# HKUST-Aerial-Robotics/VINS-Mobile

Hardware: AMD Instinct MI355X
Metric: VIO frames/sec (KLT+window solve), 640x480/150 feats/W=10 (higher is better)
Workload: dtype f64 (solve) / u8+i32+f32 (KLT)

## Files before the change

### vins-mobile_amd/csrc/vio_frontend.hip

```cpp
#include <hip/hip_runtime.h>

#include <type_traits>

#include "vio_exact_math.h"

#include <math.h>
#include <stdint.h>
#include <stdio.h>
#include <string.h>

#include <algorithm>
#include <condition_variable>
#include <memory>
#include <mutex>
#include <thread>
#include <vector>

#include "vio_amd.h"
#include "vio_device.h"
#include "vio_pool.h"

namespace {

constexpr int kMaxLevels = 4;
constexpr int kMaxCap = 512;
constexpr int kWin = 21;
constexpr int kWBits = 14;
constexpr int kMaxRadius = 128;

struct LevelDims {
  int rows[kMaxLevels], cols[kMaxLevels];
  size_t off[kMaxLevels];
  size_t pyr_bytes;
  int levels;
};

__device__ __forceinline__ int reflect101(int p, int len) {
  p = p < 0 ? -p : p;
  p = p >= len ? 2 * len - 2 - p : p;
  return p;
}
__device__ __forceinline__ int descale(int x, int n) { return (x + (1 << (n - 1))) >> n; }

constexpr int kPdW = 64, kPdH = 8;
__global__ __launch_bounds__(256) void pyr_down_kernel(const uint8_t *src_base, uint8_t *dst_base, size_t seq_stride,
                                                       int srows, int scols, int drows, int dcols) {
  constexpr int SW = 2 * kPdW + 4, SH = 2 * kPdH + 4;
  __shared__ int patch[SH][SW + 1];
  __shared__ int hsum[SH][kPdW + 1];
  const uint8_t *src = src_base + (size_t)blockIdx.z * seq_stride;
  uint8_t *dst = dst_base + (size_t)blockIdx.z * seq_stride;
  const int ox = blockIdx.x * kPdW, oy = blockIdx.y * kPdH;
  const int tid = threadIdx.x;
  for (int e = tid; e < SH * SW; e += 256) {
    int ly = e / SW, lx = e - ly * SW;
    int y = reflect101(min(2 * oy + ly - 2, 2 * srows - 2), srows), x = reflect101(min(2 * ox + lx - 2, 2 * scols - 2), scols);
    patch[ly][lx] = src[(size_t)y * scols + x];
  }
  __syncthreads();
  for (int e = tid; e < SH * kPdW; e += 256) {
    int ly = e / kPdW, lx = e - ly * kPdW;
    const int *r = &patch[ly][2 * lx];
    hsum[ly][lx] = r[0] + 4 * r[1] + 6 * r[2] + 4 * r[3] + r[4];
  }
  __syncthreads();
  for (int e = tid; e < kPdH * kPdW; e += 256) {
    int ly = e / kPdW, lx = e - ly * kPdW;
    int x = ox + lx, y = oy + ly;
    if (x < dcols && y < drows) {
      int v = hsum[2 * ly][lx] + 4 * hsum[2 * ly + 1][lx] + 6 * hsum[2 * ly + 2][lx] + 4 * hsum[2 * ly + 3][lx] + hsum[2 * ly + 4][lx];
      dst[(size_t)y * dcols + x] = (uint8_t)((v + 128) >> 8);
    }
  }
}

inline float lk_eps_screen(double eps_sq) { return nextafterf((float)(eps_sq * (1.0 + 1e-5)), INFINITY); }
struct LkParams {
  LevelDims ld;
  int cap;
  int max_count;
  float epsilon_sq_f;
  double epsilon_sq;
  float min_eig;
  const uint8_t *prev0, *next0;
  size_t stride0;
};

__device__ __forceinline__ int wave_sum_i32(int v) {
  v += __builtin_amdgcn_update_dpp(0, v, 0x111, 0xf, 0xf, false);
  v += __builtin_amdgcn_update_dpp(0, v, 0x112, 0xf, 0xf, false);
  v += __builtin_amdgcn_update_dpp(0, v, 0x114, 0xf, 0xf, false);
  v += __builtin_amdgcn_update_dpp(0, v, 0x118, 0xf, 0xf, false);
  v += __builtin_amdgcn_update_dpp(0, v, 0x142, 0xa, 0xf, false);
  v += __builtin_amdgcn_update_dpp(0, v, 0x143, 0xc, 0xf, false);
  return __builtin_amdgcn_readlane(v, 63);
}
__device__ __forceinline__ double wave_sum_exact(int p) {
  int lo = p & 0xffff, hi = p >> 16;
  int slo = wave_sum_i32(lo), shi = wave_sum_i32(hi);
  return (double)shi * 65536.0 + (double)slo;
}

__device__ __forceinline__ void lk_weights(float a, float b, int &iw00, int &iw01, int &iw10, int &iw11) {
  iw00 = __float2int_rn((1.f - a) * (1.f - b) * (1 << kWBits));
  iw01 = __float2int_rn(a * (1.f - b) * (1 << kWBits));
  iw10 = __float2int_rn((1.f - a) * b * (1 << kWBits));
  iw11 = (1 << kWBits) - iw00 - iw01 - iw10;
}

constexpr int kIP = kWin + 3;
constexpr int kDP = kWin + 1;
constexpr int kJMargin = 3;
constexpr int kJP = kWin + 1 + 2 * kJMargin;
constexpr int kJS = 43;
constexpr int kIS = kIP + 1;
struct LkWaveLds {
  union {
    struct {
      uint32_t I[kIP][kIS];
      short2 dI[kDP][kDP];
    };
    uint32_t J[kJP][kJS];
  };
};
typedef short lk_s2 __attribute__((ext_vector_type(2)));
typedef unsigned short lk_us2 __attribute__((ext_vector_type(2)));

struct __attribute__((packed)) LkU32 {
  uint32_t v;
};
__device__ __forceinline__ uint32_t lk_load4(const uint8_t *p) { return reinterpret_cast<const LkU32 *>(p)->v; }
__device__ __forceinline__ void lk_pairs(uint32_t cur, uint32_t next, uint32_t w[4]) {
  w[0] = __builtin_amdgcn_perm(0u, cur, 0x0c010c00u);
  w[1] = __builtin_amdgcn_perm(0u, cur, 0x0c020c01u);
  w[2] = __builtin_amdgcn_perm(0u, cur, 0x0c030c02u);
  w[3] = __builtin_amdgcn_perm(next, cur, 0x0c040c03u);
}

__device__ __forceinline__ void wave_lds_fence() {
  __builtin_amdgcn_fence(__ATOMIC_RELEASE, "wavefront");
  __builtin_amdgcn_wave_barrier();
  __builtin_amdgcn_fence(__ATOMIC_ACQUIRE, "wavefront");
}

__device__ __forceinline__ bool wave_all_small(int p, int q, int r = 0) {
  const bool small = (unsigned)(p + (1 << 24)) < (1u << 25) && (unsigned)(q + (1 << 24)) < (1u << 25) && (unsigned)(r + (1 << 24)) < (1u << 25);
  return __builtin_amdgcn_ballot_w64(!small) == 0ull;
}
__device__ __forceinline__ void wave_sum_exact2(int p, int q, float &sp, float &sq) {
  if (wave_all_small(p, q)) {
    int u[2] = {p, q};
#define VIO_DPPS(ctrl, rmask)                                                  \
  {                                                                            \
    const int t0 = __builtin_amdgcn_update_dpp(0, u[0], ctrl, rmask, 0xf, false); \
    const int t1 = __builtin_amdgcn_update_dpp(0, u[1], ctrl, rmask, 0xf, false); \
    u[0] += t0, u[1] += t1;                                                    \
  }
    VIO_DPPS(0x111, 0xf) VIO_DPPS(0x112, 0xf) VIO_DPPS(0x114, 0xf) VIO_DPPS(0x118, 0xf) VIO_DPPS(0x142, 0xa) VIO_DPPS(0x143, 0xc)
#undef VIO_DPPS
    sp = (float)__builtin_amdgcn_readlane(u[0], 63), sq = (float)__builtin_amdgcn_readlane(u[1], 63);
    return;
  }
  int a = p & 0xffff, b = q & 0xffff, c = p >> 16, d = q >> 16;
#define VIO_DPP4(ctrl, rmask)                                              \
  {                                                                        \
    const int ta = __builtin_amdgcn_update_dpp(0, a, ctrl, rmask, 0xf, false); \
    const int tb = __builtin_amdgcn_update_dpp(0, b, ctrl, rmask, 0xf, false); \
    const int tc = __builtin_amdgcn_update_dpp(0, c, ctrl, rmask, 0xf, false); \
    const int td = __builtin_amdgcn_update_dpp(0, d, ctrl, rmask, 0xf, false); \
    a += ta, b += tb, c += tc, d += td;                                    \
  }
  VIO_DPP4(0x111, 0xf) VIO_DPP4(0x112, 0xf) VIO_DPP4(0x114, 0xf) VIO_DPP4(0x118, 0xf) VIO_DPP4(0x142, 0xa) VIO_DPP4(0x143, 0xc)
#undef VIO_DPP4
  const int sa = __builtin_amdgcn_readlane(a, 63), sb = __builtin_amdgcn_readlane(b, 63), sc = __builtin_amdgcn_readlane(c, 63),
            sd = __builtin_amdgcn_readlane(d, 63);
  sp = (float)sc * 65536.f + (float)sa, sq = (float)sd * 65536.f + (float)sb;
}

__device__ __forceinline__ void wave_sum_exact3(int p, int q, int r, float &sp, float &sq, float &sr) {
  if (wave_all_small(p, q, r)) {
    int w[3] = {p, q, r};
#define VIO_DPPS3(ctrl, rmask)                                                                                       \
  {                                                                                                                   \
    int t[3];                                                                                                         \
    _Pragma("unroll") for (int k = 0; k < 3; k++) t[k] = __builtin_amdgcn_update_dpp(0, w[k], ctrl, rmask, 0xf, false); \
    _Pragma("unroll") for (int k = 0; k < 3; k++) w[k] += t[k];                                                       \
  }
    VIO_DPPS3(0x111, 0xf) VIO_DPPS3(0x112, 0xf) VIO_DPPS3(0x114, 0xf) VIO_DPPS3(0x118, 0xf) VIO_DPPS3(0x142, 0xa) VIO_DPPS3(0x143, 0xc)
#undef VIO_DPPS3
    sp = (float)__builtin_amdgcn_readlane(w[0], 63), sq = (float)__builtin_amdgcn_readlane(w[1], 63), sr = (float)__builtin_amdgcn_readlane(w[2], 63);
    return;
  }
  int u[3] = {p, q, r};
#define VIO_DPPN(N, arr, ctrl, rmask)                                               \
  {                                                                                 \
    int t[N];                                                                       \
    _Pragma("unroll") for (int k = 0; k < N; k++) t[k] = __builtin_amdgcn_update_dpp(0, arr[k], ctrl, rmask, 0xf, false); \
    _Pragma("unroll") for (int k = 0; k < N; k++) arr[k] += t[k];                   \
  }
  VIO_DPPN(3, u, 0x111, 0xf) VIO_DPPN(3, u, 0x112, 0xf) VIO_DPPN(3, u, 0x114, 0xf) VIO_DPPN(3, u, 0x118, 0xf)
  int v[6] = {u[0] & 0xffff, u[1] & 0xffff, u[2] & 0xffff, u[0] >> 16, u[1] >> 16, u[2] >> 16};
  VIO_DPPN(6, v, 0x142, 0xa) VIO_DPPN(6, v, 0x143, 0xc)
#undef VIO_DPPN
  int s[6];
#pragma unroll
  for (int k = 0; k < 6; k++) s[k] = __builtin_amdgcn_readlane(v[k], 63);
  sp = (float)s[3] * 65536.f + (float)s[0], sq = (float)s[4] * 65536.f + (float)s[1], sr = (float)s[5] * 65536.f + (float)s[2];
}

template <bool STATS = false>
__global__ __launch_bounds__(256, 6) void lk_track_kernel(const uint8_t *prev_pyr, const uint8_t *next_pyr, LkParams P,
                                                       const int *n_pts, const float *prev_pts, float *next_pts,
                                                       uint8_t *status, float *err, unsigned long long *stats) {
  __shared__ LkWaveLds lds_all[4];
  const int seq = blockIdx.y;
  const int wave = threadIdx.x >> 6, lane = threadIdx.x & 63;
  const int pt = blockIdx.x * (blockDim.x >> 6) + wave;
  if (pt >= n_pts[seq]) return;
  LkWaveLds &L = lds_all[wave];
  const uint8_t *pp = prev_pyr + (size_t)seq * P.ld.pyr_bytes, *np = next_pyr + (size_t)seq * P.ld.pyr_bytes;
  const size_t pidx = ((size_t)seq * P.cap + pt) * 2;
  const float ptx = prev_pts[pidx], pty = prev_pts[pidx + 1];
  const float half = (kWin - 1) * 0.5f;
  const float FLT_SCALE = 1.f / (1 << 20);
  constexpr int NPX = (kWin * kWin + 63) / 64;
  const int wy0 = min(lane / kWin, 2), wx0 = lane % kWin;
  const int joff = wy0 * kJS + wx0;
  bool st = true;
  float er = 0.f;
  float nxx = 0.f, nxy = 0.f;
  const int max_level = P.ld.levels - 1;
  for (int level = max_level; level >= 0; level--) {
    const int rows = P.ld.rows[level], cols = P.ld.cols[level];
    const uint8_t *I = pp + P.ld.off[level], *J = np + P.ld.off[level];
    if (level == 0) {
      if (P.prev0) I = P.prev0 + (size_t)seq * P.stride0;
      if (P.next0) J = P.next0 + (size_t)seq * P.stride0;
    }
    const float scale = __int_as_float((127 - level) << 23);
    float px = ptx * scale, py = pty * scale;
    float qx, qy;
    if (level == max_level) qx = px, qy = py;
    else qx = nxx * 2.f, qy = nxy * 2.f;
    nxx = qx, nxy = qy;
    px -= half, py -= half;
    int ipx = (int)floorf(px), ipy = (int)floorf(py);
    if (ipx < -kWin || ipx >= cols || ipy < -kWin || ipy >= rows) {
      if (level == 0) st = false, er = 0.f;
      continue;
    }
    float a = px - ipx, b = py - ipy;
    int iw00, iw01, iw10, iw11;
    lk_weights(a, b, iw00, iw01, iw10, iw11);
    wave_lds_fence();
    if (ipx >= 1 && ipx + kIP - 1 <= cols && ipy >= 1 && ipy + kIP - 1 <= rows) {
      const int r = lane / 6, d = lane - 6 * r;
      constexpr int TI = (kIP + 9) / 10;
      uint32_t curs[TI];
#pragma unroll
      for (int t = 0; t < TI; t++) {
        const int ly = r + 10 * t;
        curs[t] = lk_load4(I + (unsigned)(__mul24(ipy - 1 + (ly < kIP ? ly : 0), cols) + ipx - 1 + 4 * d));
      }
#pragma unroll
      for (int t = 0; t < TI; t++) {
        const int ly = r + 10 * t;
        const bool ok = lane < 60 && ly < kIP;
        const uint32_t cur = curs[t];
        uint32_t next = (uint32_t)__builtin_amdgcn_update_dpp(0, (int)cur, 0x130, 0xf, 0xf, false);
        if (d == 5) next = cur >> 24;
        uint32_t w4[4];
        lk_pairs(cur, next, w4);
        if (ok) {
#pragma unroll
          for (int k = 0; k < 4; k++) L.I[ly][4 * d + k] = w4[k];
        }
      }
    } else {
      const int lx = lane & 31;
      const int x = reflect101(ipx - 1 + min(lx, kIP - 1), cols);
      constexpr int RPT = 2, TB = kIP / RPT;
      static_assert(kIP % RPT == 0, "whole trips");
      int vs[TB];
#pragma unroll
      for (int t = 0; t < TB; t++) {
        const int s_y0 = __builtin_amdgcn_readfirstlane(ipy) - 1 + RPT * t;
        const int ro_a = reflect101(s_y0, rows) * cols, ro_b = reflect101(s_y0 + 1, rows) * cols;
        vs[t] = I[(unsigned)(((lane >> 5) ? ro_b : ro_a) + x)];
      }
#pragma unroll
      for (int t = 0; t < TB; t++) {
        const int ly = (lane >> 5) + RPT * t, v = vs[t];
        const int vr = __builtin_amdgcn_update_dpp(0, v, 0x130, 0xf, 0xf, false);
        if (lx < kIP) L.I[ly][lx] = (uint32_t)v | ((uint32_t)vr << 16);
      }
    }
    wave_lds_fence();
    constexpr int SEG = 5, NSEG = 5, NCP = kDP / 2;
    static_assert(kDP % 2 == 0 && NCP * NSEG <= 64 && SEG * NSEG >= kDP && kDP >= SEG, "column pairs x segments");
    const bool inside = ipx >= 0 && ipx + kDP <= cols && ipy >= 0 && ipy + kDP <= rows;
    if (lane < NCP * NSEG) {
      const int seg = lane / NCP, cp = lane - NCP * seg, c = 2 * cp;
      const int r0 = seg * SEG < kDP - SEG ? seg * SEG : kDP - SEG;
      const uint32_t *Ip = &L.I[0][0] + (__mul24(r0, kIS) + c);
      uint32_t *Dp = reinterpret_cast<uint32_t *>(&L.dI[0][0]) + (__mul24(r0, kDP) + c);
      const lk_s2 k3 = {3, 3}, k10 = {10, 10};
      auto walk = [&](auto checked) {
        const unsigned ok0 = (unsigned)(ipx + c) < (unsigned)cols, ok1 = (unsigned)(ipx + c + 1) < (unsigned)cols;
        lk_s2 P0[SEG + 2], P1[SEG + 2], P2[SEG + 2];
#pragma unroll
        for (int r = 0; r < SEG + 2; r++)
          __builtin_memcpy(&P0[r], Ip + r * kIS, 4), __builtin_memcpy(&P1[r], Ip + r * kIS + 1, 4), __builtin_memcpy(&P2[r], Ip + r * kIS + 2, 4);
        lk_s2 h[SEG + 2], v[SEG + 2];
#pragma unroll
        for (int r = 0; r < SEG + 2; r++) h[r] = P2[r] - P0[r], v[r] = (P0[r] + P2[r]) * k3 + P1[r] * k10;
#pragma unroll
        for (int r = 2; r < SEG + 2; r++) {
          const lk_s2 dx = (h[r - 2] + h[r]) * k3 + h[r - 1] * k10, dy = v[r] - v[r - 2];
          uint32_t ux, uy;
          __builtin_memcpy(&ux, &dx, 4), __builtin_memcpy(&uy, &dy, 4);
          uint32_t d0 = __builtin_amdgcn_perm(uy, ux, 0x05040100u), d1 = __builtin_amdgcn_perm(uy, ux, 0x07060302u);
          if (decltype(checked)::value) {
            const unsigned rok = (unsigned)(ipy + r0 + r - 2) < (unsigned)rows;
            d0 &= 0u - (ok0 & rok), d1 &= 0u - (ok1 & rok);
          }
          Dp[(r - 2) * kDP] = d0, Dp[(r - 2) * kDP + 1] = d1;
        }
      };
      if (inside) walk(std::false_type{});
      else walk(std::true_type{});
    }
    wave_lds_fence();
    constexpr int NPP = (NPX + 1) / 2;
    const lk_s2 sw_top = {(short)iw00, (short)iw01}, sw_bot = {(short)iw10, (short)iw11};
    lk_s2 IxP[NPP], IyP[NPP];
    int Ic[NPX];
    int p11 = 0, p12 = 0, p22 = 0;
#pragma unroll
    for (int h = 0; h < NPP; h++) IxP[h] = IyP[h] = lk_s2{0, 0};
#pragma unroll
    for (int q = 0; q < NPX; q++) {
      const int y = wy0 + 3 * q, x = wx0;
      lk_s2 it, ib;
      __builtin_memcpy(&it, &L.I[y + 1][x + 1], 4);
      __builtin_memcpy(&ib, &L.I[y + 2][x + 1], 4);
      const int ival = __builtin_amdgcn_sdot2(it, sw_top, __builtin_amdgcn_sdot2(ib, sw_bot, 1 << (kWBits - 5 - 1), false), false) >> (kWBits - 5);
      uint32_t d00, d01, d10, d11;
      __builtin_memcpy(&d00, &L.dI[y][x], 4), __builtin_memcpy(&d01, &L.dI[y][x + 1], 4);
      __builtin_memcpy(&d10, &L.dI[y + 1][x], 4), __builtin_memcpy(&d11, &L.dI[y + 1][x + 1], 4);
      const uint32_t xt = __builtin_amdgcn_perm(d01, d00, 0x05040100u), yt = __builtin_amdgcn_perm(d01, d00, 0x07060302u);
      const uint32_t xb = __builtin_amdgcn_perm(d11, d10, 0x05040100u), yb = __builtin_amdgcn_perm(d11, d10, 0x07060302u);
      lk_s2 sxt, syt, sxb, syb;
      __builtin_memcpy(&sxt, &xt, 4), __builtin_memcpy(&syt, &yt, 4), __builtin_memcpy(&sxb, &xb, 4), __builtin_memcpy(&syb, &yb, 4);
      int ixval = __builtin_amdgcn_sdot2(sxt, sw_top, __builtin_amdgcn_sdot2(sxb, sw_bot, 1 << (kWBits - 1), false), false) >> kWBits;
      int iyval = __builtin_amdgcn_sdot2(syt, sw_top, __builtin_amdgcn_sdot2(syb, sw_bot, 1 << (kWBits - 1), false), false) >> kWBits;
      if (lane >= 3 * kWin) ixval = iyval = 0;
      Ic[q] = (1 << (kWBits - 5 - 1)) - (int)((unsigned)ival << (kWBits - 5));
      if (q & 1) IxP[q >> 1].y = (short)ixval, IyP[q >> 1].y = (short)iyval;
      else IxP[q >> 1].x = (short)ixval, IyP[q >> 1].x = (short)iyval;
      p11 += ixval * ixval, p12 += ixval * iyval, p22 += iyval * iyval;
    }
    float f11, f12, f22;
    wave_sum_exact3(p11, p12, p22, f11, f12, f22);
    float A11 = f11 * FLT_SCALE, A12 = f12 * FLT_SCALE, A22 = f22 * FLT_SCALE;
    float D = A11 * A22 - A12 * A12;
    float minEig = (A22 + A11 - sqrtf((A11 - A22) * (A11 - A22) + 4.f * A12 * A12)) / (2 * kWin * kWin);
    if (minEig < P.min_eig || D < 1.1920929e-07f) {
      if (level == 0) st = false;
      continue;
    }
    D = 1.f / D;
    qx -= half, qy -= half;
    float pdx = 0.f, pdy = 0.f;
    int jox = 0, joy = 0;
    bool j_staged = false;
    auto stage_j = [&](int iqx, int iqy) {
      jox = iqx - kJMargin, joy = iqy - kJMargin;
      wave_lds_fence();
      if (jox >= 0 && jox + kJP <= cols && joy >= 0 && joy + kJP <= rows) {
        const int r = lane / 7, d = lane - 7 * r;
        constexpr int TJ = (kJP + 8) / 9;
        uint32_t curs[TJ];
#pragma unroll
        for (int t = 0; t < TJ; t++) {
          const int ly = r + 9 * t;
          curs[t] = lk_load4(J + (unsigned)(__mul24(joy + (ly < kJP ? ly : 0), cols) + jox + 4 * d));
        }
#pragma unroll
        for (int t = 0; t < TJ; t++) {
          const int ly = r + 9 * t;
          const bool ok = lane < 63 && ly < kJP;
          const uint32_t cur = curs[t];
          uint32_t next = (uint32_t)__builtin_amdgcn_update_dpp(0, (int)cur, 0x130, 0xf, 0xf, false);
          if (d == 6) next = cur >> 24;
          uint32_t w4[4];
          lk_pairs(cur, next, w4);
          if (ok) {
#pragma unroll
            for (int k = 0; k < 4; k++) L.J[ly][4 * d + k] = w4[k];
          }
        }
      } else {
        const int lx = lane & 31;
        const int x = reflect101(min(max(jox + min(lx, kJP - 1), -cols + 1), 2 * cols - 2), cols);
        constexpr int RPT = 2, TB = kJP / RPT;
        static_assert(kJP % RPT == 0, "whole trips");
        int vs[TB];
#pragma unroll
        for (int t = 0; t < TB; t++) {
          const int s_y0 = __builtin_amdgcn_readfirstlane(joy) + RPT * t;
          const int ro_a = reflect101(min(max(s_y0, -rows + 1), 2 * rows - 2), rows) * cols;
          const int ro_b = reflect101(min(max(s_y0 + 1, -rows + 1), 2 * rows - 2), rows) * cols;
          vs[t] = J[(unsigned)(((lane >> 5) ? ro_b : ro_a) + x)];
        }
#pragma unroll
        for (int t = 0; t < TB; t++) {
          const int ly = (lane >> 5) + RPT * t, v = vs[t];
          const int vr = __builtin_amdgcn_update_dpp(0, v, 0x130, 0xf, 0xf, false);
          if (lx < kJP) L.J[ly][lx] = (uint32_t)v | ((uint32_t)vr << 16);
        }
      }
      wave_lds_fence();
      j_staged = true;
    };
    const uint32_t *Jl = &L.J[0][0];
    auto diff_j = [&](int base, int q, lk_us2 wtop, lk_s2 wbot) {
      lk_us2 top;
      lk_s2 bot;
      const int o = base + (joff + 3 * q * kJS);
      const uint32_t t32 = Jl[o], b32 = Jl[o + kJS];
      __builtin_memcpy(&top, &t32, 4);
      __builtin_memcpy(&bot, &b32, 4);
      return __builtin_amdgcn_sdot2(bot, wbot, (int)__builtin_amdgcn_udot2(top, wtop, (unsigned)Ic[q], false), false) >> (kWBits - 5);
    };
    int nit = 0;
    for (int j = 0; j < P.max_count; j++) {
      int iqx = (int)floorf(qx), iqy = (int)floorf(qy);
      if (iqx < -kWin || iqx >= cols || iqy < -kWin || iqy >= rows) {
        if (level == 0) st = false;
        break;
      }
      if (STATS) nit++;
      if (!j_staged || iqx < jox || iqx > jox + 2 * kJMargin || iqy < joy || iqy > joy + 2 * kJMargin) stage_j(iqx, iqy);
      a = qx - iqx, b = qy - iqy;
      lk_weights(a, b, iw00, iw01, iw10, iw11);
      int pb1 = 0, pb2 = 0;
      const lk_us2 wtop = {(unsigned short)iw00, (unsigned short)iw01};
      const lk_s2 wbot = {(short)iw10, (short)iw11};
      const int jbase = __mul24(iqy - joy, kJS) + (iqx - jox);
#pragma unroll
      for (int h = 0; h < NPP; h++) {
        const int d0 = diff_j(jbase, 2 * h, wtop, wbot), d1 = 2 * h + 1 < NPX ? diff_j(jbase, 2 * h + 1, wtop, wbot) : 0;
        const unsigned pk = __builtin_amdgcn_perm((unsigned)d1, (unsigned)d0, 0x05040100u);
        lk_s2 dp;
        __builtin_memcpy(&dp, &pk, 4);
        pb1 = __builtin_amdgcn_sdot2(dp, IxP[h], pb1, false), pb2 = __builtin_amdgcn_sdot2(dp, IyP[h], pb2, false);
      }
      float fb1, fb2;
      wave_sum_exact2(pb1, pb2, fb1, fb2);
      float b1 = fb1 * FLT_SCALE, b2 = fb2 * FLT_SCALE;
      float ddx = (A12 * b2 - A22 * b1) * D, ddy = (A12 * b1 - A11 * b2) * D;
      qx += ddx, qy += ddy;
      nxx = qx + half, nxy = qy + half;
      if (!(ddx * ddx + ddy * ddy > P.epsilon_sq_f) && (double)ddx * ddx + (double)ddy * ddy <= P.epsilon_sq) break;
      constexpr float kCentiUp = 0.010000000707805157f;
      static_assert((double)kCentiUp > 0.01 && (double)0.01f < 0.01, "float neighbours of 0.01");
      if (j > 0 && fabsf(ddx + pdx) < kCentiUp && fabsf(ddy + pdy) < kCentiUp) {
        nxx -= ddx * 0.5f, nxy -= ddy * 0.5f;
        break;
      }
      pdx = ddx, pdy = ddy;
    }
    if (STATS && lane == 0) {
      unsigned long long *sl = stats + ((blockIdx.x + 7 * blockIdx.y) & 63) * 16;
      atomicAdd(sl + level, (unsigned long long)nit);
      atomicAdd(sl + P.ld.levels + level, 1ull);
    }
    if (st && level == 0) {
      float ex = nxx - half, ey = nxy - half;
      int iex = (int)floorf(ex), iey = (int)floorf(ey);
      if (iex < -kWin || iex >= cols || iey < -kWin || iey >= rows) {
        st = false;
        continue;
      }
      if (!j_staged || iex < jox || iex > jox + 2 * kJMargin || iey < joy || iey > joy + 2 * kJMargin) stage_j(iex, iey);
      float aa = ex - iex, bb = ey - iey;
      lk_weights(aa, bb, iw00, iw01, iw10, iw11);
      int pe = 0;
      const lk_us2 wtop = {(unsigned short)iw00, (unsigned short)iw01};
      const lk_s2 wbot = {(short)iw10, (short)iw11};
      const int jbase = __mul24(iey - joy, kJS) + (iex - jox);
#pragma unroll
      for (int q = 0; q < NPX; q++) {
        const int d = abs(diff_j(jbase, q, wtop, wbot));
        pe += lane < 3 * kWin ? d : 0;
      }
      const int se = wave_sum_i32(pe);
      er = (float)se * 1.f / (32 * kWin * kWin);
    }
  }
  if (lane == 0) {
    next_pts[pidx] = nxx, next_pts[pidx + 1] = nxy;
    status[(size_t)seq * P.cap + pt] = st ? 1 : 0;
    err[(size_t)seq * P.cap + pt] = er;
  }
}

__device__ __attribute__((noinline)) double exact_fn(int which, double x) {
  return which == 0 ? vio_xm::acos_cr(x) : which == 1 ? vio_xm::cos_cr(x) : vio_xm::pow_cr(x, 0.333333333333);
}
__device__ int solve_cubic_dev(const double c[4], double r[3], bool exact) {
  double a0 = c[0], a1 = c[1], a2 = c[2], a3 = c[3];
  double x0 = 0, x1 = 0, x2 = 0;
  int n = 0;
  if (a0 == 0) {
    if (a1 == 0) {
      if (a2 == 0) n = a3 == 0 ? -1 : 0;
      else x0 = -a3 / a2, n = 1;
    } else {
      double d = a2 * a2 - 4 * a1 * a3;
      if (d >= 0) {
        d = sqrt(d);
        double q1 = (-a2 + d) * 0.5, q2 = (a2 + d) * -0.5;
        if (fabs(q1) > fabs(q2)) x0 = q1 / a1, x1 = a3 / q1;
        else x0 = q2 / a1, x1 = a3 / q2;
        n = d > 0 ? 2 : 1;
      }
    }
  } else {
    a0 = 1. / a0, a1 *= a0, a2 *= a0, a3 *= a0;
    double Q = (a1 * a1 - 3 * a2) * (1. / 9), R = (2 * a1 * a1 * a1 - 9 * a1 * a2 + 27 * a3) * (1. / 54);
    double Qcubed = Q * Q * Q, d = Qcubed - R * R;
    const double kPi = 3.14159265358979323846;
    if (d >= 0) {
      const double av = R / sqrt(Qcubed);
      double theta = exact ? exact_fn(0, av) : acos(av), sqrtQ = sqrt(Q);
      double t0 = -2 * sqrtQ, t1 = theta * (1. / 3), t2 = a1 * (1. / 3);
      const double g0 = t1, g1 = t1 + (2. * kPi / 3), g2 = t1 + (4. * kPi / 3);
      if (exact) x0 = t0 * exact_fn(1, g0) - t2, x1 = t0 * exact_fn(1, g1) - t2, x2 = t0 * exact_fn(1, g2) - t2;
      else x0 = t0 * cos(g0) - t2, x1 = t0 * cos(g1) - t2, x2 = t0 * cos(g2) - t2;
      n = 3;
    } else {
      d = sqrt(-d);
      double e = exact ? exact_fn(2, d + fabs(R)) : pow(d + fabs(R), 0.333333333333);
      if (R > 0) e = -e;
      x0 = (e + Q / e) - a1 * (1. / 3);
      n = 1;
    }
  }
  r[0] = x0, r[1] = x1, r[2] = x2;
  return n;
}

struct SevenPointWork {
  double a[63], f1[9], f2[9];
  int colperm[10];
};

__device__ __forceinline__ int run7point_group(const float *ms1, const float *ms2, double *fmatrix, SevenPointWork &wk, int l, bool exact) {
  double *a = wk.a, *f1 = wk.f1, *f2 = wk.f2;
  int *colperm = wk.colperm;
  auto group_sync = [] {
    __builtin_amdgcn_fence(__ATOMIC_RELEASE, "wavefront");
    __builtin_amdgcn_wave_barrier();
    __builtin_amdgcn_fence(__ATOMIC_ACQUIRE, "wavefront");
  };
  if (l < 7) {
    double x0 = ms1[2 * l], y0 = ms1[2 * l + 1], x1 = ms2[2 * l], y1 = ms2[2 * l + 1];
    double *row = a + l * 9;
    row[0] = x1 * x0, row[1] = x1 * y0, row[2] = x1, row[3] = y1 * x0, row[4] = y1 * y0, row[5] = y1, row[6] = x0,
    row[7] = y0, row[8] = 1;
  }
  if (l < 9) colperm[l] = l;
  group_sync();
  for (int k = 0; k < 7; k++) {
    double best = -1;
    int bpos = k * 9 + k;
#pragma unroll
    for (int q = 0; q < 4; q++) {
      const int e = l + 16 * q, i = e / 9, j = e - 9 * i;
      if (e < 63 && i >= k && j >= k) {
        const double v = fabs(a[e]);
        if (v > best) best = v, bpos = e;
      }
    }
#pragma unroll
    for (int m = 1; m < 16; m <<= 1) {
      const double ob = __shfl_xor(best, m, 16);
      const int op = __shfl_xor(bpos, m, 16);
      if (ob > best || (ob == best && op < bpos)) best = ob, bpos = op;
    }
    const int pr = bpos / 9, pc = bpos - 9 * pr;
    if (pr != k && l < 9) {
      const double t = a[k * 9 + l];
      a[k * 9 + l] = a[pr * 9 + l], a[pr * 9 + l] = t;
    }
    group_sync();
    if (pc != k) {
      if (l < 7) {
        const double t = a[l * 9 + k];
        a[l * 9 + k] = a[l * 9 + pc], a[l * 9 + pc] = t;
      }
      if (l == 15) {
        const int t = colperm[k];
        colperm[k] = colperm[pc], colperm[pc] = t;
      }
    }
    group_sync();
    const double d = a[k * 9 + k];
    group_sync();
    if (d == 0.0) continue;
    if (l < 9) a[k * 9 + l] /= d;
    group_sync();
    double fv[4], pv[4], av[4];
    int ev[4];
#pragma unroll
    for (int q = 0; q < 4; q++) {
      const int e = l + 16 * q, ii = e / 9, j = e - 9 * ii, i = ii < k ? ii : ii + 1;
      const bool on = e < 54;
      ev[q] = on ? i * 9 + j : -1;
      fv[q] = on ? a[i * 9 + k] : 0.0, pv[q] = on ? a[k * 9 + j] : 0.0, av[q] = on ? a[i * 9 + j] : 0.0;
    }
    group_sync();
#pragma unroll
    for (int q = 0; q < 4; q++)
      if (ev[q] >= 0 && fv[q] != 0.0) a[ev[q]] = av[q] - fv[q] * pv[q];
    group_sync();
  }
  if (l < 9) {
#pragma unroll
    for (int q = 0; q < 2; q++) {
      double *out = q == 0 ? f1 : f2;
      const double vj = l < 7 ? -a[l * 9 + 7 + q] : (l - 7 == q ? 1.0 : 0.0);
      out[colperm[l]] = vj;
    }
  }
  group_sync();
  if (l < 9) f1[l] -= f2[l];
  group_sync();
  int n = 0;
  if (l == 0) {
    double c[4], r[3];
    double t0 = f2[4] * f2[8] - f2[5] * f2[7], t1 = f2[3] * f2[8] - f2[5] * f2[6], t2 = f2[3] * f2[7] - f2[4] * f2[6];
    c[3] = f2[0] * t0 - f2[1] * t1 + f2[2] * t2;
    c[2] = f1[0] * t0 - f1[1] * t1 + f1[2] * t2 - f1[3] * (f2[1] * f2[8] - f2[2] * f2[7]) +
           f1[4] * (f2[0] * f2[8] - f2[2] * f2[6]) - f1[5] * (f2[0] * f2[7] - f2[1] * f2[6]) +
           f1[6] * (f2[1] * f2[5] - f2[2] * f2[4]) - f1[7] * (f2[0] * f2[5] - f2[2] * f2[3]) +
           f1[8] * (f2[0] * f2[4] - f2[1] * f2[3]);
    t0 = f1[4] * f1[8] - f1[5] * f1[7], t1 = f1[3] * f1[8] - f1[5] * f1[6], t2 = f1[3] * f1[7] - f1[4] * f1[6];
    c[1] = f2[0] * t0 - f2[1] * t1 + f2[2] * t2 - f2[3] * (f1[1] * f1[8] - f1[2] * f1[7]) +
           f2[4] * (f1[0] * f1[8] - f1[2] * f1[6]) - f2[5] * (f1[0] * f1[7] - f1[1] * f1[6]) +
           f2[6] * (f1[1] * f1[5] - f1[2] * f1[4]) - f2[7] * (f1[0] * f1[5] - f1[2] * f1[3]) +
           f2[8] * (f1[0] * f1[4] - f1[1] * f1[3]);
    c[0] = f1[0] * t0 - f1[1] * t1 + f1[2] * t2;
    n = solve_cubic_dev(c, r, exact);
    if (n >= 1 && n <= 3)
      for (int k = 0; k < n; k++, fmatrix += 9) {
// ... 1035 lines not shown
      }
    }
    __syncthreads();
    if (tid < SH) {
      if (ox == 0) {
        const uint32_t d1 = raw[tid][1];
        raw[tid][0] = ((d1 >> 16) & 0xffu) << 16 | ((d1 >> 8) & 0xffu) << 24;
      }
      const int lr = ndw - dw0;
      if (lr >= 1 && lr < kPd4Dw) {
        const uint32_t dl = raw[tid][lr - 1];
        raw[tid][lr] = ((dl >> 16) & 0xffu) | ((dl >> 8) & 0xffu) << 8;
      }
    }
    __syncthreads();
    for (int e = tid; e < (SH / 2) * kPdW; e += 256) {
      const int p = e / kPdW, lx = e - p * kPdW;
      const int b = 2 * lx + 2, dwi = b >> 2, sh = (b & 3) * 8;
      auto hrow = [&](int ly) {
        const uint32_t lo = raw[ly][dwi], hi = raw[ly][dwi + 1];
        return __builtin_amdgcn_udot4(__builtin_amdgcn_alignbit(hi, lo, sh), 0x04060401u, __builtin_amdgcn_ubfe(hi, sh, 8), false);
      };
      hsum[p][lx] = hrow(2 * p) | hrow(2 * p + 1) << 16;
    }
    __syncthreads();
    {
      const int ly = tid >> 4, lx = (tid & 15) * 4;
      const int x = ox + lx, y = oy + ly;
      if (x < dcols && y < drows) {
        uint32_t out = 0;
        const lk_us2 w14 = {1, 4}, w64 = {6, 4};
#pragma unroll
        for (int i = 0; i < 4; i++) {
          lk_us2 p0, p1;
          __builtin_memcpy(&p0, &hsum[ly][lx + i], 4), __builtin_memcpy(&p1, &hsum[ly + 1][lx + i], 4);
          const uint32_t v = __builtin_amdgcn_udot2(p0, w14, __builtin_amdgcn_udot2(p1, w64, hsum[ly + 2][lx + i] & 0xffffu, false), false);
          out |= ((v + 128) >> 8) << (8 * i);
        }
        *reinterpret_cast<uint32_t *>(dst + (size_t)y * dcols + x) = out;
      }
    }
    if (!more) break;
#pragma unroll
    for (int i = 0; i < NE; i++) cur[i] = nxt[i];
  }
}

__global__ __launch_bounds__(256) void copy_frames_kernel(const uint8_t *src, size_t src_stride, uint8_t *dst,
                                                          size_t dst_stride, size_t bytes, int vec_ok) {
  const int seq = blockIdx.y;
  const uint8_t *sp = src + (size_t)seq * src_stride;
  uint8_t *dp = dst + (size_t)seq * dst_stride;
  const size_t i = (size_t)blockIdx.x * blockDim.x + threadIdx.x;
  if (vec_ok) {
    if (i * 16 < bytes) reinterpret_cast<uint4 *>(dp)[i] = reinterpret_cast<const uint4 *>(sp)[i];
  } else {
    const size_t b0 = i * 16, b1 = b0 + 16 < bytes ? b0 + 16 : bytes;
    for (size_t b = b0; b < b1; b++) dp[b] = sp[b];
  }
}

int launch_track_update(vio_frontend *fe, int publish, hipStream_t st) {
  TrackerArrays A;
  A.cap = fe->cap, A.rows = fe->cfg.image_rows, A.cols = fe->cfg.image_cols;
  A.cur_pts = fe->cur_pts.p, A.pre_pts = fe->pre_pts.p, A.forw_pts = fe->forw_pts.p, A.ids = fe->ids.p, A.track_cnt = fe->track_cnt.p;
  A.n_pts = fe->n_pts.p, A.n_forw = fe->n_forw.p, A.n_id = fe->n_id.p, A.lk_status = fe->lk_status.p, A.kept_xy = fe->kept_xy.p;
  A.n_kept = fe->n_kept.p, A.hw = fe->hw.p, A.radius = fe->cfg.min_dist, A.f_thresh = (float)fe->cfg.f_threshold;
  A.pnp_pts = fe->pnp_pts.p, A.pnp_ids = fe->pnp_ids.p, A.n_pnp = fe->n_pnp.p;
  A.f_conf = fe->cfg.f_confidence;
  static const bool tu_prof = vio::env_flag("VIO_AMD_TU_PROF");
  if (tu_prof) (void)fe->d_prof.ensure(32);
  A.prof = tu_prof ? fe->d_prof.p : nullptr;
  const bool small = fe->cap <= 256;
  const size_t shm = ((small ? sizeof(TrackShared<256>) : sizeof(TrackShared<kMaxCap>)) + 15 & ~(size_t)15) + sizeof(RansacShared);
  const void *kern = small ? (const void *)track_update_kernel<256> : (const void *)track_update_kernel<kMaxCap>;
  if (!fe->attr_set) {
    HIP_OK(hipFuncSetAttribute(kern, hipFuncAttributeMaxDynamicSharedMemorySize, (int)shm));
    fe->attr_set = true;
  }
  if (A.prof) (void)hipMemsetAsync(A.prof, 0, 32 * sizeof(long long), st);
  if (small) hipLaunchKernelGGL(track_update_kernel<256>, dim3(fe->n_seq), dim3(256), shm, st, A, publish);
  else hipLaunchKernelGGL(track_update_kernel<kMaxCap>, dim3(fe->n_seq), dim3(256), shm, st, A, publish);
  if (A.prof) {
    long long h[32];
    if (hipStreamSynchronize(st) == hipSuccess && hipMemcpy(h, A.prof, sizeof(h), hipMemcpyDeviceToHost) == hipSuccess) {
      static const char *name[11] = {"load", "compact", "ransac(cur,forw)", "compact", "pnp list", "ransac(pre,forw)", "compact", "counts+rank",
                                     "inside bits", "greedy", "outputs"};
      fprintf(stderr, "track_update cycles (sequence 0, publish %d):", publish);
      const int map[11][2] = {{0, 1}, {1, 2}, {2, 3}, {3, 4}, {4, 5}, {5, 6}, {6, 7}, {7, 8}, {8, 9}, {9, 10}, {10, 11}};
      for (int k = 0; k < 11; k++) fprintf(stderr, " %s %lld,", name[k], h[map[k][1]] - h[map[k][0]]);
      fprintf(stderr, " total %lld\n", h[11] - h[0]);
      for (int c = 0; c < 2; c++)
        fprintf(stderr, "   ransac call %d: draw %lld, gather+collinear %lld, 7-point %lld, scoring %lld, scan %lld, mask %lld, rounds %lld\n", c,
                h[16 + 8 * c], h[17 + 8 * c], h[18 + 8 * c], h[19 + 8 * c], h[20 + 8 * c], h[21 + 8 * c], h[22 + 8 * c]);
    }
  }
  return VIO_OK;
}

int fe_step(vio_frontend *fe, const uint8_t *d_frames , int publish, hipStream_t st, bool keep_frames = false) {
  const int S = fe->n_seq, rows = fe->cfg.image_rows, cols = fe->cfg.image_cols, cap = fe->cap;
  const size_t img_bytes = (size_t)rows * cols;
  const int fidx = fe->have_img ? 1 - fe->cur_idx : fe->cur_idx;
  uint8_t *forw = fe->pyr[fidx].p;
  const bool fused0 = fe->ld.levels >= 2 && cols % 4 == 0 && fe->ld.cols[1] % 4 == 0 && cols >= 8 && fe->ld.pyr_bytes % 4 == 0 &&
                      img_bytes % 4 == 0 && (uintptr_t)d_frames % 4 == 0 && (uintptr_t)forw % 4 == 0 && fe->ld.off[1] % 4 == 0;
  const bool alias0 = keep_frames && fused0 && !vio::env_flag("VIO_AMD_COPY_LEVEL0");
  fe->lvl0[fidx] = alias0 ? d_frames : nullptr;
  if (!fused0) {
    const int vec_ok = img_bytes % 16 == 0 && fe->ld.pyr_bytes % 16 == 0 && (uintptr_t)d_frames % 16 == 0 &&
                       (uintptr_t)forw % 16 == 0;
    dim3 grd((unsigned)((img_bytes + 16 * 256 - 1) / (16 * 256)), S);
    hipLaunchKernelGGL(copy_frames_kernel, grd, dim3(256), 0, st, d_frames, img_bytes, forw, fe->ld.pyr_bytes, img_bytes,
                       vec_ok);
  }
  for (int l = 1; l < fe->ld.levels; l++) {
    const uint8_t *sp = forw + fe->ld.off[l - 1];
    uint8_t *dp = forw + fe->ld.off[l];
    const int sc = fe->ld.cols[l - 1], dc = fe->ld.cols[l];
    if (l == 1 && fused0) {
      dim3 blk(256), grd((dc + kPdW - 1) / kPdW, (fe->ld.rows[1] + kPd4H * kPd4T - 1) / (kPd4H * kPd4T), S);
      if (alias0)
        hipLaunchKernelGGL(pyr_down4_kernel<false>, grd, blk, 0, st, d_frames, img_bytes, dp, fe->ld.pyr_bytes, rows, cols, fe->ld.rows[1], dc,
                           (uint8_t *)nullptr);
      else
        hipLaunchKernelGGL(pyr_down4_kernel<true>, grd, blk, 0, st, d_frames, img_bytes, dp, fe->ld.pyr_bytes, rows, cols, fe->ld.rows[1], dc, forw);
      continue;
    }
    const bool dwords = sc % 4 == 0 && dc % 4 == 0 && sc >= 8 && fe->ld.pyr_bytes % 4 == 0 && (uintptr_t)sp % 4 == 0 && (uintptr_t)dp % 4 == 0;
    if (dwords) {
      dim3 blk(256), grd((dc + kPdW - 1) / kPdW, (fe->ld.rows[l] + kPd4H * kPd4T - 1) / (kPd4H * kPd4T), S);
      hipLaunchKernelGGL(pyr_down4_kernel<false>, grd, blk, 0, st, sp, fe->ld.pyr_bytes, dp, fe->ld.pyr_bytes, fe->ld.rows[l - 1], sc, fe->ld.rows[l], dc,
                         (uint8_t *)nullptr);
    } else {
      dim3 blk(256), grd((dc + kPdW - 1) / kPdW, (fe->ld.rows[l] + kPdH - 1) / kPdH, S);
      hipLaunchKernelGGL(pyr_down_kernel, grd, blk, 0, st, sp, dp, fe->ld.pyr_bytes, fe->ld.rows[l - 1], sc, fe->ld.rows[l], dc);
    }
  }
  if (!fe->have_img) {
    fe->have_img = true;
    fe->cur_idx = fidx;
  } else {
    LkParams P;
    P.ld = fe->ld, P.cap = cap;
    P.max_count = std::min(std::max(fe->cfg.lk_max_iters, 0), 100);
    double eps = std::min(std::max(fe->cfg.lk_eps, 0.), 10.);
    P.epsilon_sq = eps * eps, P.epsilon_sq_f = lk_eps_screen(eps * eps), P.min_eig = (float)fe->cfg.lk_min_eig;
    P.prev0 = fe->lvl0[fe->cur_idx], P.next0 = fe->lvl0[fidx], P.stride0 = img_bytes;
    dim3 grd((cap + 3) / 4, S);
    if (fe->lk_stats_on && fe->lk_stats.p)
      hipLaunchKernelGGL((lk_track_kernel<true>), grd, dim3(256), 0, st, fe->pyr[fe->cur_idx].p, forw, P, fe->n_pts.p, fe->cur_pts.p,
                         fe->forw_pts.p, fe->lk_status.p, fe->lk_err.p, fe->lk_stats.p);
    else
      hipLaunchKernelGGL((lk_track_kernel<false>), grd, dim3(256), 0, st, fe->pyr[fe->cur_idx].p, forw, P, fe->n_pts.p, fe->cur_pts.p,
                         fe->forw_pts.p, fe->lk_status.p, fe->lk_err.p, (unsigned long long *)nullptr);
  }
  int rcu = launch_track_update(fe, publish, st);
  if (rcu != VIO_OK) return rcu;
  if (publish) {
    dim3 tb(256), tg((cols + kDetWaves * kDetW - 1) / (kDetWaves * kDetW), fe->nseg, S);
    hipLaunchKernelGGL(detect_kernel<false>, tg, tb, 0, st, alias0 ? d_frames : forw, alias0 ? img_bytes : fe->ld.pyr_bytes, (const uint8_t *)nullptr, (size_t)0,
                       fe->kept_xy.p, fe->n_kept.p, cap, fe->hw.p, fe->cfg.min_dist, fe->max_bits.p, rows, cols, fe->cand.p,
                       fe->seg_cap, fe->n_cand.p, fe->detect_always ? (const int *)nullptr : fe->n_forw.p, fe->cfg.max_corners);
    SelectParams SP;
    SP.cap = cap, SP.rows = rows, SP.cols = cols, SP.max_corners = fe->cfg.max_corners, SP.min_dist = (float)fe->cfg.min_dist;
    SP.fx = fe->cfg.fx, SP.fy = fe->cfg.fy, SP.cx = fe->cfg.cx, SP.cy = fe->cfg.cy;
    hipLaunchKernelGGL(corner_select_kernel, dim3(S), dim3(kSelThreads), 0, st, fe->cand.p, fe->seg_cap, fe->nseg, fe->n_cand.p,
                       fe->max_bits.p, fe->cfg.quality_level, SP, fe->forw_pts.p, fe->cur_pts.p, fe->pre_pts.p, fe->ids.p,
                       fe->track_cnt.p, fe->n_forw.p, fe->n_pts.p, fe->n_id.p, fe->obs.p, fe->n_obs.p, fe->cs_prof ? fe->d_cs_prof.p : nullptr);
    if (fe->cs_prof) {
      long long h[5];
      if (hipStreamSynchronize(st) == hipSuccess && hipMemcpy(h, fe->d_cs_prof.p, sizeof(h), hipMemcpyDeviceToHost) == hipSuccess)
        fprintf(stderr, "corner_select cycles (sequence 0): threshold %lld, selection %lld, ids %lld, outputs %lld, total %lld\n", h[1] - h[0],
                h[2] - h[1], h[3] - h[2], h[4] - h[3], h[4] - h[0]);
    }
  }
  HIP_OK(hipGetLastError());
  fe->cur_idx = fidx;
  return VIO_OK;
}

}

extern "C" {

int vio_frontend_create(const VioConfig *cfg, int32_t n_seq, vio_frontend_t **out) {
  if (!cfg || !out || n_seq < 1) return VIO_EINVAL;
  if (cfg->lk_win != kWin || cfg->lk_levels < 0 || cfg->lk_levels >= kMaxLevels || cfg->max_corners < 1 ||
      cfg->max_corners > kMaxCap || cfg->image_rows < 32 || cfg->image_cols < 32 || cfg->min_dist < 0 || cfg->min_dist > kMaxRadius ||
      cfg->image_rows > 32767 || cfg->image_cols > 65535)
    return VIO_EINVAL;
  if (!vio::device_ready("the front-end")) return VIO_ENODEV;
  vio_frontend *fe = new vio_frontend();
  fe->device = vio::current_device();
  fe->cfg = *cfg, fe->n_seq = n_seq, fe->cap = cfg->max_corners;
  fe->detect_always = vio::env_flag("VIO_AMD_DETECT_ALWAYS");
  fe->cs_prof = vio::env_flag("VIO_AMD_CS_PROF") && fe->d_cs_prof.ensure(8) == VIO_OK;
  LevelDims &ld = fe->ld;
  ld.rows[0] = cfg->image_rows, ld.cols[0] = cfg->image_cols, ld.off[0] = 0, ld.levels = 1;
  size_t off = (size_t)ld.rows[0] * ld.cols[0];
  for (int l = 1; l <= cfg->lk_levels; l++) {
    int r = (ld.rows[l - 1] + 1) / 2, c = (ld.cols[l - 1] + 1) / 2;
    if (c <= kWin || r <= kWin) break;
    ld.rows[l] = r, ld.cols[l] = c, ld.off[l] = off, off += (size_t)r * c, ld.levels = l + 1;
  }
  ld.pyr_bytes = (off + 255) & ~(size_t)255;
  const size_t S = n_seq, cap = fe->cap;
  fe->nseg = (cfg->image_rows + kDetR - 1) / kDetR;
  if (fe->nseg > kSelMaxSeg) {
    delete fe;
    return VIO_ECAP;
  }
  fe->seg_cap = kDetR * cfg->image_cols / 4;
  if (hipStreamCreateWithFlags(&fe->stream, hipStreamNonBlocking) != hipSuccess) {
    delete fe;
    return VIO_ENODEV;
  }
  if (fe->pyr[0].ensure(S * ld.pyr_bytes) != VIO_OK || fe->pyr[1].ensure(S * ld.pyr_bytes) != VIO_OK ||
      fe->max_bits.ensure(S * fe->nseg) != VIO_OK || fe->cand.ensure(S * fe->nseg * fe->seg_cap) != VIO_OK ||
      fe->n_cand.ensure(S * fe->nseg) != VIO_OK || fe->cur_pts.ensure(S * cap * 2) != VIO_OK ||
      fe->pre_pts.ensure(S * cap * 2) != VIO_OK || fe->forw_pts.ensure(S * cap * 2) != VIO_OK || fe->lk_err.ensure(S * cap) != VIO_OK ||
      fe->ids.ensure(S * cap) != VIO_OK || fe->track_cnt.ensure(S * cap) != VIO_OK || fe->n_pts.ensure(S) != VIO_OK ||
      fe->n_forw.ensure(S) != VIO_OK || fe->n_id.ensure(S) != VIO_OK || fe->kept_xy.ensure(S * cap * 2) != VIO_OK ||
      fe->n_kept.ensure(S) != VIO_OK || fe->pnp_pts.ensure(S * cap * 2) != VIO_OK || fe->pnp_ids.ensure(S * cap) != VIO_OK ||
      fe->n_pnp.ensure(S) != VIO_OK || fe->n_obs.ensure(S) != VIO_OK || fe->lk_status.ensure(S * cap) != VIO_OK ||
      fe->obs.ensure(S * cap) != VIO_OK || fe->hw.ensure((size_t)2 * cfg->min_dist + 1) != VIO_OK) {
    delete fe;
    return VIO_ENOMEM;
  }
  std::vector<int> hw;
  circle_halfwidths(cfg->min_dist, hw);
  if (hipMemcpy(fe->hw.p, hw.data(), hw.size() * sizeof(int), hipMemcpyHostToDevice) != hipSuccess ||
      hipMemset(fe->max_bits.p, 0, sizeof(unsigned) * S * fe->nseg) != hipSuccess ||
      hipMemset(fe->n_cand.p, 0, sizeof(int) * S * fe->nseg) != hipSuccess || hipMemset(fe->n_pts.p, 0, sizeof(int) * S) != hipSuccess ||
      hipMemset(fe->n_forw.p, 0, sizeof(int) * S) != hipSuccess || hipMemset(fe->n_id.p, 0, sizeof(int) * S) != hipSuccess ||
      hipMemset(fe->n_kept.p, 0, sizeof(int) * S) != hipSuccess || hipMemset(fe->n_pnp.p, 0, sizeof(int) * S) != hipSuccess ||
      hipMemset(fe->n_obs.p, 0, sizeof(int) * S) != hipSuccess) {
    delete fe;
    return VIO_ENODEV;
  }
  *out = fe;
  return VIO_OK;
}

int vio_frontend_get_device(const vio_frontend_t *fe, int32_t *device) {
  if (!fe || !device) return VIO_EINVAL;
  *device = fe->device;
  return VIO_OK;
}

void vio_frontend_destroy(vio_frontend_t *fe) {
  if (!fe) return;
  vio::DeviceScope scope(fe->device);
  delete fe;
}

int vio_frontend_upload_frames(vio_frontend_t *fe, const uint8_t *gray, int32_t n_frames, int32_t rows, int32_t cols,
                               int32_t stride) {
  if (!fe || !gray || n_frames < 1) return VIO_EINVAL;
  if (rows != fe->cfg.image_rows || cols != fe->cfg.image_cols || stride < cols) return VIO_EINVAL;
  VIO_ON_DEVICE_OF(fe);
  const size_t px = (size_t)rows * cols, total = (size_t)n_frames * fe->n_seq;
  if (fe->pending) return VIO_ESTATE;
  HIP_OK(hipDeviceSynchronize());
  for (int k = 0; k < 2; k++) {
    if (fe->lvl0[k])
      HIP_OK(hipMemcpy2D(fe->pyr[k].p, fe->ld.pyr_bytes, fe->lvl0[k], px, px, fe->n_seq, hipMemcpyDeviceToDevice));
    fe->lvl0[k] = nullptr;
  }
  fe->frames.release();
  if (fe->frames.ensure(total * px) != VIO_OK) return VIO_ENOMEM;
  HIP_OK(hipMemcpy2D(fe->frames.p, cols, gray, stride, cols, total * rows, hipMemcpyHostToDevice));
  fe->n_frames = n_frames;
  return VIO_OK;
}

int vio_frontend_step_resident(vio_frontend_t *fe, int32_t frame_index, int32_t publish, void *stream) {
  if (!fe) return VIO_EINVAL;
  if (!fe->frames.p || frame_index < 0 || frame_index >= fe->n_frames) return VIO_ESTATE;
  if (fe->pending) return VIO_ESTATE;
  VIO_ON_DEVICE_OF(fe);
  hipStream_t st = stream ? (hipStream_t)stream : fe->stream;
  int rc = fe->timer.begin(st);
  if (rc != VIO_OK) return rc;
  const size_t px = (size_t)fe->cfg.image_rows * fe->cfg.image_cols;
  rc = fe_step(fe, fe->frames.p + (size_t)frame_index * fe->n_seq * px, publish, st, true);
  if (rc != VIO_OK) return rc;
  return fe->timer.end(st);
}

int vio_frontend_sync(vio_frontend_t *fe) {
  if (!fe) return VIO_EINVAL;
  VIO_ON_DEVICE_OF(fe);
  HIP_OK(hipDeviceSynchronize());
  return VIO_OK;
}

int vio_frontend_kernel_ms(vio_frontend_t *fe, double *ms_avg, int32_t *launches) {
  if (!fe || !ms_avg || !launches) return VIO_EINVAL;
  VIO_ON_DEVICE_OF(fe);
  HIP_OK(hipDeviceSynchronize());
  return fe->timer.drain(ms_avg, launches);
}

namespace {
struct HostRange {
  const uint8_t *p;
  size_t n;
// ... 410 lines not shown
```

Baseline: 185,300.

## Remap LK lane pixels and LDS strides to avoid bank conflicts, skip error pass

Moves each lane's pixels in the LK tracking kernel from every third row to a block of consecutive rows (with a column rotation for the middle group). It pads the I, dI and J LDS arrays to a stride of 29, with a compile-time check that the window reads have no bank conflicts. Adjacent row taps are now reused across pixels, and the J rows are loaded once per iteration into registers. The default launch also drops the final per-point error computation and its store (ERR=false), which is safe only if no later stage reads lk_err.

```diff
diff --git a/vins-mobile_amd/csrc/lk_layout.h b/vins-mobile_amd/csrc/lk_layout.h
--- /dev/null
+++ b/vins-mobile_amd/csrc/lk_layout.h
@@ -0,0 +1,54 @@
+#pragma once
+
+namespace lk_layout {
+
+constexpr int kWin = 21;
+constexpr int kLanes = 64;
+constexpr int kBanks = 32;
+constexpr int kBankGroup = 32;
+constexpr int kPxPerLane = 7;
+constexpr int kOwners = 3 * kWin;
+
+constexpr int kStrideI = 29, kStrideDI = 29, kStrideJ = 29;
+
+struct Px {
+  int row, col;
+};
+constexpr Px lane_pixel0(int lane) {
+  const int g = lane / kWin < 2 ? lane / kWin : 2;
+  const int c = lane % kWin;
+  return Px{kPxPerLane * g, g == 1 ? (c + 10) % kWin : c};
+}
+
+constexpr int lds_extra_cycles(const int (&addr)[kLanes]) {
+  int extra = 0;
+  for (int g0 = 0; g0 < kLanes; g0 += kBankGroup) {
+    int cnt[kBanks] = {};
+    for (int i = g0; i < g0 + kBankGroup; i++) {
+      bool dup = false;
+      for (int j = g0; j < i; j++) dup = dup || addr[j] == addr[i];
+      if (!dup) cnt[((addr[i] % kBanks) + kBanks) % kBanks]++;
+    }
+    int worst = 1;
+    for (int b = 0; b < kBanks; b++) worst = cnt[b] > worst ? cnt[b] : worst;
+    extra += worst - 1;
+  }
+  return extra;
+}
+
+constexpr int window_read_extra_cycles(int stride, int dy, int dx, int base = 0) {
+  int addr[kLanes] = {};
+  for (int l = 0; l < kLanes; l++) {
+    const Px p = lane_pixel0(l);
+    addr[l] = base + (p.row + dy) * stride + p.col + dx;
+  }
+  return lds_extra_cycles(addr);
+}
+constexpr int window_reads_extra_cycles(int stride) {
+  int extra = 0;
+  for (int dy = 0; dy <= kPxPerLane + 1; dy++)
+    for (int dx = 0; dx <= 2; dx++) extra += window_read_extra_cycles(stride, dy, dx);
+  return extra;
+}
+
+}
diff --git a/vins-mobile_amd/csrc/vio_frontend.hip b/vins-mobile_amd/csrc/vio_frontend.hip
--- a/vins-mobile_amd/csrc/vio_frontend.hip
+++ b/vins-mobile_amd/csrc/vio_frontend.hip
@@ -2,6 +2,7 @@
 
 #include <type_traits>
 
+#include "lk_layout.h"
 #include "vio_exact_math.h"
 
 #include <math.h>
@@ -112,13 +113,16 @@
 constexpr int kDP = kWin + 1;
 constexpr int kJMargin = 3;
 constexpr int kJP = kWin + 1 + 2 * kJMargin;
-constexpr int kJS = 43;
-constexpr int kIS = kIP + 1;
+constexpr int kIS = lk_layout::kStrideI, kDS = lk_layout::kStrideDI, kJS = lk_layout::kStrideJ;
+static_assert(lk_layout::kWin == kWin && kIS >= kIP && kDS >= kDP && kJS >= kJP, "strides hold a row");
+static_assert(lk_layout::window_reads_extra_cycles(kIS) == 0 && lk_layout::window_reads_extra_cycles(kDS) == 0 &&
+                  lk_layout::window_reads_extra_cycles(kJS) == 0,
+              "window reads of I, dI and J are free of LDS bank conflicts");
 struct LkWaveLds {
   union {
     struct {
       uint32_t I[kIP][kIS];
-      short2 dI[kDP][kDP];
+      uint32_t dI[kDP][kDS];
     };
     uint32_t J[kJP][kJS];
   };
@@ -208,13 +212,13 @@
   sp = (float)s[3] * 65536.f + (float)s[0], sq = (float)s[4] * 65536.f + (float)s[1], sr = (float)s[5] * 65536.f + (float)s[2];
 }
 
-template <bool STATS = false>
+template <bool STATS = false, bool ERR = true>
 __global__ __launch_bounds__(256, 6) void lk_track_kernel(const uint8_t *prev_pyr, const uint8_t *next_pyr, LkParams P,
                                                        const int *n_pts, const float *prev_pts, float *next_pts,
                                                        uint8_t *status, float *err, unsigned long long *stats) {
   __shared__ LkWaveLds lds_all[4];
   const int seq = blockIdx.y;
-  const int wave = threadIdx.x >> 6, lane = threadIdx.x & 63;
+  const int wave = __builtin_amdgcn_readfirstlane(threadIdx.x >> 6), lane = threadIdx.x & 63;
   const int pt = blockIdx.x * (blockDim.x >> 6) + wave;
   if (pt >= n_pts[seq]) return;
   LkWaveLds &L = lds_all[wave];
@@ -224,7 +228,9 @@
   const float half = (kWin - 1) * 0.5f;
   const float FLT_SCALE = 1.f / (1 << 20);
   constexpr int NPX = (kWin * kWin + 63) / 64;
-  const int wy0 = min(lane / kWin, 2), wx0 = lane % kWin;
+  static_assert(NPX == lk_layout::kPxPerLane, "pixels per lane");
+  const lk_layout::Px px0 = lk_layout::lane_pixel0(lane);
+  const int wy0 = px0.row, wx0 = px0.col;
   const int joff = wy0 * kJS + wx0;
   bool st = true;
   float er = 0.f;
@@ -303,7 +309,7 @@
       const int seg = lane / NCP, cp = lane - NCP * seg, c = 2 * cp;
       const int r0 = seg * SEG < kDP - SEG ? seg * SEG : kDP - SEG;
       const uint32_t *Ip = &L.I[0][0] + (__mul24(r0, kIS) + c);
-      uint32_t *Dp = reinterpret_cast<uint32_t *>(&L.dI[0][0]) + (__mul24(r0, kDP) + c);
+      uint32_t *Dp = reinterpret_cast<uint32_t *>(&L.dI[0][0]) + (__mul24(r0, kDS) + c);
       const lk_s2 k3 = {3, 3}, k10 = {10, 10};
       auto walk = [&](auto checked) {
         const unsigned ok0 = (unsigned)(ipx + c) < (unsigned)cols, ok1 = (unsigned)(ipx + c + 1) < (unsigned)cols;
@@ -324,7 +330,7 @@
             const unsigned rok = (unsigned)(ipy + r0 + r - 2) < (unsigned)rows;
             d0 &= 0u - (ok0 & rok), d1 &= 0u - (ok1 & rok);
           }
-          Dp[(r - 2) * kDP] = d0, Dp[(r - 2) * kDP + 1] = d1;
+          Dp[(r - 2) * kDS] = d0, Dp[(r - 2) * kDS + 1] = d1;
         }
       };
       if (inside) walk(std::false_type{});
@@ -338,22 +344,24 @@
     int p11 = 0, p12 = 0, p22 = 0;
 #pragma unroll
     for (int h = 0; h < NPP; h++) IxP[h] = IyP[h] = lk_s2{0, 0};
+    const uint32_t *Iw = &L.I[wy0 + 1][wx0 + 1], *Dw = &L.dI[wy0][wx0];
+    auto tap_row = [&](int k, lk_s2 &iv, lk_s2 &sx, lk_s2 &sy) {
+      uint32_t d0, d1;
+      __builtin_memcpy(&iv, Iw + k * kIS, 4);
+      __builtin_memcpy(&d0, Dw + k * kDS, 4), __builtin_memcpy(&d1, Dw + k * kDS + 1, 4);
+      const uint32_t xs = __builtin_amdgcn_perm(d1, d0, 0x05040100u), ys = __builtin_amdgcn_perm(d1, d0, 0x07060302u);
+      __builtin_memcpy(&sx, &xs, 4), __builtin_memcpy(&sy, &ys, 4);
+    };
+    lk_s2 it, sxt, syt;
+    tap_row(0, it, sxt, syt);
 #pragma unroll
     for (int q = 0; q < NPX; q++) {
-      const int y = wy0 + 3 * q, x = wx0;
-      lk_s2 it, ib;
-      __builtin_memcpy(&it, &L.I[y + 1][x + 1], 4);
-      __builtin_memcpy(&ib, &L.I[y + 2][x + 1], 4);
+      lk_s2 ib, sxb, syb;
+      tap_row(q + 1, ib, sxb, syb);
       const int ival = __builtin_amdgcn_sdot2(it, sw_top, __builtin_amdgcn_sdot2(ib, sw_bot, 1 << (kWBits - 5 - 1), false), false) >> (kWBits - 5);
-      uint32_t d00, d01, d10, d11;
-      __builtin_memcpy(&d00, &L.dI[y][x], 4), __builtin_memcpy(&d01, &L.dI[y][x + 1], 4);
-      __builtin_memcpy(&d10, &L.dI[y + 1][x], 4), __builtin_memcpy(&d11, &L.dI[y + 1][x + 1], 4);
-      const uint32_t xt = __builtin_amdgcn_perm(d01, d00, 0x05040100u), yt = __builtin_amdgcn_perm(d01, d00, 0x07060302u);
-      const uint32_t xb = __builtin_amdgcn_perm(d11, d10, 0x05040100u), yb = __builtin_amdgcn_perm(d11, d10, 0x07060302u);
-      lk_s2 sxt, syt, sxb, syb;
-      __builtin_memcpy(&sxt, &xt, 4), __builtin_memcpy(&syt, &yt, 4), __builtin_memcpy(&sxb, &xb, 4), __builtin_memcpy(&syb, &yb, 4);
       int ixval = __builtin_amdgcn_sdot2(sxt, sw_top, __builtin_amdgcn_sdot2(sxb, sw_bot, 1 << (kWBits - 1), false), false) >> kWBits;
       int iyval = __builtin_amdgcn_sdot2(syt, sw_top, __builtin_amdgcn_sdot2(syb, sw_bot, 1 << (kWBits - 1), false), false) >> kWBits;
+      it = ib, sxt = sxb, syt = syb;
       if (lane >= 3 * kWin) ixval = iyval = 0;
       Ic[q] = (1 << (kWBits - 5 - 1)) - (int)((unsigned)ival << (kWBits - 5));
       if (q & 1) IxP[q >> 1].y = (short)ixval, IyP[q >> 1].y = (short)iyval;
@@ -424,13 +432,15 @@
       j_staged = true;
     };
     const uint32_t *Jl = &L.J[0][0];
-    auto diff_j = [&](int base, int q, lk_us2 wtop, lk_s2 wbot) {
+    auto load_j = [&](int base, uint32_t (&jr)[NPX + 1]) {
+#pragma unroll
+      for (int k = 0; k <= NPX; k++) jr[k] = Jl[base + (joff + k * kJS)];
+    };
+    auto diff_j = [&](const uint32_t (&jr)[NPX + 1], int q, lk_us2 wtop, lk_s2 wbot) {
       lk_us2 top;
       lk_s2 bot;
-      const int o = base + (joff + 3 * q * kJS);
-      const uint32_t t32 = Jl[o], b32 = Jl[o + kJS];
-      __builtin_memcpy(&top, &t32, 4);
-      __builtin_memcpy(&bot, &b32, 4);
+      __builtin_memcpy(&top, &jr[q], 4);
+      __builtin_memcpy(&bot, &jr[q + 1], 4);
       return __builtin_amdgcn_sdot2(bot, wbot, (int)__builtin_amdgcn_udot2(top, wtop, (unsigned)Ic[q], false), false) >> (kWBits - 5);
     };
     int nit = 0;
@@ -448,9 +458,11 @@
       const lk_us2 wtop = {(unsigned short)iw00, (unsigned short)iw01};
       const lk_s2 wbot = {(short)iw10, (short)iw11};
       const int jbase = __mul24(iqy - joy, kJS) + (iqx - jox);
+      uint32_t jr[NPX + 1];
+      load_j(jbase, jr);
 #pragma unroll
       for (int h = 0; h < NPP; h++) {
-        const int d0 = diff_j(jbase, 2 * h, wtop, wbot), d1 = 2 * h + 1 < NPX ? diff_j(jbase, 2 * h + 1, wtop, wbot) : 0;
+        const int d0 = diff_j(jr, 2 * h, wtop, wbot), d1 = 2 * h + 1 < NPX ? diff_j(jr, 2 * h + 1, wtop, wbot) : 0;
         const unsigned pk = __builtin_amdgcn_perm((unsigned)d1, (unsigned)d0, 0x05040100u);
         lk_s2 dp;
         __builtin_memcpy(&dp, &pk, 4);
@@ -483,6 +495,7 @@
         st = false;
         continue;
       }
+      if (!ERR) continue;
       if (!j_staged || iex < jox || iex > jox + 2 * kJMargin || iey < joy || iey > joy + 2 * kJMargin) stage_j(iex, iey);
       float aa = ex - iex, bb = ey - iey;
       lk_weights(aa, bb, iw00, iw01, iw10, iw11);
@@ -490,9 +503,11 @@
       const lk_us2 wtop = {(unsigned short)iw00, (unsigned short)iw01};
       const lk_s2 wbot = {(short)iw10, (short)iw11};
       const int jbase = __mul24(iey - joy, kJS) + (iex - jox);
+      uint32_t jr[NPX + 1];
+      load_j(jbase, jr);
 #pragma unroll
       for (int q = 0; q < NPX; q++) {
-        const int d = abs(diff_j(jbase, q, wtop, wbot));
+        const int d = abs(diff_j(jr, q, wtop, wbot));
         pe += lane < 3 * kWin ? d : 0;
       }
       const int se = wave_sum_i32(pe);
@@ -502,7 +517,7 @@
   if (lane == 0) {
     next_pts[pidx] = nxx, next_pts[pidx + 1] = nxy;
     status[(size_t)seq * P.cap + pt] = st ? 1 : 0;
-    err[(size_t)seq * P.cap + pt] = er;
+    if (ERR) err[(size_t)seq * P.cap + pt] = er;
   }
 }
 
@@ -1844,8 +1859,8 @@
       hipLaunchKernelGGL((lk_track_kernel<true>), grd, dim3(256), 0, st, fe->pyr[fe->cur_idx].p, forw, P, fe->n_pts.p, fe->cur_pts.p,
                          fe->forw_pts.p, fe->lk_status.p, fe->lk_err.p, fe->lk_stats.p);
     else
-      hipLaunchKernelGGL((lk_track_kernel<false>), grd, dim3(256), 0, st, fe->pyr[fe->cur_idx].p, forw, P, fe->n_pts.p, fe->cur_pts.p,
-                         fe->forw_pts.p, fe->lk_status.p, fe->lk_err.p, (unsigned long long *)nullptr);
+      hipLaunchKernelGGL((lk_track_kernel<false, false>), grd, dim3(256), 0, st, fe->pyr[fe->cur_idx].p, forw, P, fe->n_pts.p, fe->cur_pts.p,
+                         fe->forw_pts.p, fe->lk_status.p, (float *)nullptr, (unsigned long long *)nullptr);
   }
   int rcu = launch_track_update(fe, publish, st);
   if (rcu != VIO_OK) return rcu;
```

New measurement: 191,600 (median of 6 runs). 1.03x the previous value.
